# NiteshBharadwaj/pytorch-unsup-pc

Measured on AMD Instinct MI355X. Metric: point-clouds/sec (8000 pts->64^3->128^2 proj) fwd+bwd, higher is better.
Workload: dtype f32

## Files before the change

pytorch-unsup-pc_amd/csrc/dpc_common.h:

```cpp
#pragma once
#include <hip/hip_runtime.h>
#include <stdint.h>

#include "../../include/dpc_render.h"

#define DPC_WAVE 64

template <int RB>
struct TapsT {
  float w[2 * RB + 1];
};

struct TapsDyn {
  float w[DPC_MAX_TAPS];
  int n;
};

template <int RB>
__device__ inline TapsT<RB> resolve_taps(const TapsT<RB>& host, const float* __restrict__ dev, int n, bool flip) {
  if (dev == nullptr || n <= 0) return host;
  TapsT<RB> t;
  const int c = (n - 1) / 2;
#pragma unroll
  for (int i = 0; i < 2 * RB + 1; ++i) {
// ... 94 lines not shown
  for (int i = 0; i < 9; ++i) g.m[i] = 0.f;
  g.dt[0] = g.dt[1] = g.dt[2] = 0.f;
  g.df = 0.f;
}

__device__ inline void project_point_bwd(const Camera& c, const Projected& o, float px, float py, float pz, float dZ,
                                         float dY, float dX, float& dpx, float& dpy, float& dpz, CamGrad& g) {
  const float g2 = c.f * o.inv * dX;
  const float g1 = c.f * o.inv * dY;
  const float persp = -(o.X * dX + o.Y * dY) * o.inv;
  const float g0 = dZ + persp;
  g.df += (o.p2 * dX + o.p1 * dY) * o.inv;
  g.dt[0] += persp;
  g.dt[1] += g1;
  g.dt[2] += g2;
  dpx = fmaf(c.r[0], g0, fmaf(c.r[3], g1, c.r[6] * g2));
  dpy = fmaf(c.r[1], g0, fmaf(c.r[4], g1, c.r[7] * g2));
  dpz = fmaf(c.r[2], g0, fmaf(c.r[5], g1, c.r[8] * g2));
  g.m[0] += px * g0; g.m[1] += px * g1; g.m[2] += px * g2;
  g.m[3] += py * g0; g.m[4] += py * g1; g.m[5] += py * g2;
  g.m[6] += pz * g0; g.m[7] += pz * g1; g.m[8] += pz * g2;
}

__device__ inline void quaternion_grad(const Camera& c, const float* m, float* dq) {
  const float w = c.qw, vx = c.qx, vy = c.qy, vz = c.qz;
  const float tr = m[0] + m[4] + m[8];
  const float cx = m[5] - m[7], cy = m[6] - m[2], cz = m[1] - m[3];
  const float sx = 2.f * m[0] * vx + (m[1] + m[3]) * vy + (m[2] + m[6]) * vz;
  const float sy = (m[3] + m[1]) * vx + 2.f * m[4] * vy + (m[5] + m[7]) * vz;
  const float sz = (m[6] + m[2]) * vx + (m[7] + m[5]) * vy + 2.f * m[8] * vz;
  const float gw = 2.f * (w * tr + vx * cx + vy * cy + vz * cz);
  const float gx = 2.f * (-tr * vx + sx + w * cx);
  const float gy = 2.f * (-tr * vy + sy + w * cy);
  const float gz = 2.f * (-tr * vz + sz + w * cz);
  const float dot = w * gw + vx * gx + vy * gy + vz * gz;
  dq[0] = (gw - w * dot) * c.inv_norm;
  dq[1] = (gx - vx * dot) * c.inv_norm;
  dq[2] = (gy - vy * dot) * c.inv_norm;
  dq[3] = (gz - vz * dot) * c.inv_norm;
}

struct CameraRef {
  float w, x, y, z;
  double cw, cx, cy, cz;
  double tx, ty, tz;
  double f, d;
  bool has_t;
};

__device__ inline CameraRef load_camera_ref(const DpcParams& P, const float* __restrict__ q,
                                            const float* __restrict__ t, const float* __restrict__ f, int b) {
#pragma clang fp contract(off)
  CameraRef c;
  const float q0 = q[4 * b + 0], q1 = q[4 * b + 1], q2 = q[4 * b + 2], q3 = q[4 * b + 3];
  float acc = 0.f;
  acc = acc + q0 * q0;
  acc = acc + q1 * q1;
  acc = acc + q2 * q2;
  acc = acc + q3 * q3;
  const float n = sqrtf(acc);
  c.w = q0 / n; c.x = q1 / n; c.y = q2 / n; c.z = q3 / n;
  c.cw = (double)c.w; c.cx = -(double)c.x; c.cy = -(double)c.y; c.cz = -(double)c.z;
  c.has_t = t != nullptr;
  c.tx = t ? (double)t[3 * b + 0] : 0.0;
  c.ty = t ? (double)t[3 * b + 1] : 0.0;
  c.tz = t ? (double)t[3 * b + 2] : 0.0;
  c.f = f ? (double)f[b] : (double)P.focal_length;
  c.d = (double)P.camera_distance;
  return c;
}

__device__ inline void project_point_ref(const CameraRef& c, float x2, float y2, float z2, double& Z, double& Y,
                                         double& X) {
#pragma clang fp contract(off)
  const float w2 = 0.0f;
  const float w1 = c.w, x1 = c.x, y1 = c.y, z1 = c.z;
  const float aw = ((w1 * w2 - x1 * x2) - y1 * y2) - z1 * z2;
  const float ax = ((w1 * x2 + x1 * w2) + y1 * z2) - z1 * y2;
  const float ay = ((w1 * y2 + y1 * w2) + z1 * x2) - x1 * z2;
  const float az = ((w1 * z2 + z1 * w2) + x1 * y2) - y1 * x2;
  const double dw = (double)aw, dx = (double)ax, dy = (double)ay, dz = (double)az;
  double p0 = ((dw * c.cx + dx * c.cw) + dy * c.cz) - dz * c.cy;
  double p1 = ((dw * c.cy + dy * c.cw) + dz * c.cx) - dx * c.cz;
  double p2 = ((dw * c.cz + dz * c.cw) + dx * c.cy) - dy * c.cx;
  if (c.has_t) {
    p0 = p0 + c.tx; p1 = p1 + c.ty; p2 = p2 + c.tz;
  }
  double zs = p0 + c.d;
  const double xs = (p2 * c.f) / zs;
  const double ys = (p1 * c.f) / zs;
  zs = zs - c.d;
  if (c.has_t) zs = zs - c.tx;
  Z = zs; Y = ys; X = xs;
}

struct __attribute__((aligned(16))) PointRec {
  int code;
  float tz, ty, tx;
};

struct Cell {
  int iz, iy, ix;
  float wz[2], wy[2], wx[2];
  bool valid;
};

__device__ inline float frac_encode(double g, int& cell) {
#pragma clang fp contract(off)
  const double fl = floor(g);
  cell = (int)fl;
  const double r = g - fl;
  return (float)(r < 0.5 ? r : r - 1.0);
}

__device__ inline PointRec make_record(double Z, double Y, double X, int D, int H, int W) {
#pragma clang fp contract(off)
  PointRec rec;
  const bool valid = (Z >= -0.5) && (Z <= 0.5) && (Y >= -0.5) && (Y <= 0.5) && (X >= -0.5) && (X <= 0.5);
  int iz, iy, ix;
  rec.tz = frac_encode((Z + 0.5) * (double)(D - 1), iz);
  rec.ty = frac_encode((Y + 0.5) * (double)(H - 1), iy);
  rec.tx = frac_encode((X + 0.5) * (double)(W - 1), ix);
  rec.code = valid ? ((iz << 20) | (iy << 10) | ix) : -1;
  if (!valid) rec.tz = rec.ty = rec.tx = 0.f;
  return rec;
}

__device__ inline void frac_decode(float t, float (&w)[2]) {
  w[1] = t >= 0.f ? t : 1.0f + t;
  w[0] = t >= 0.f ? 1.0f - t : -t;
}

__device__ inline Cell cell_from_record(const PointRec& rec) {
  Cell c;
  c.valid = rec.code >= 0;
  c.iz = rec.code >> 20;
  c.iy = (rec.code >> 10) & 1023;
  c.ix = rec.code & 1023;
  frac_decode(rec.tz, c.wz);
  frac_decode(rec.ty, c.wy);
  frac_decode(rec.tx, c.wx);
  return c;
}

__device__ inline PointRec load_record(const PointRec* __restrict__ recs, size_t i) {
  const int4 v = *reinterpret_cast<const int4*>(recs + i);
  PointRec r;
  r.code = v.x;
  r.tz = __int_as_float(v.y);
  r.ty = __int_as_float(v.z);
  r.tx = __int_as_float(v.w);
  return r;
}

template <int RB, int L, bool CLAMP1>
__device__ inline void window_load(float (&v)[L + 2 * RB], const float* base, int stride, int start, int len) {
#pragma unroll
  for (int i = 0; i < L + 2 * RB; ++i) {
    const int pos = start + i - RB;
    float x = (pos >= 0 && pos < len) ? base[pos * stride] : 0.f;
    if (CLAMP1) x = fminf(x, 1.0f);
    v[i] = x;
  }
}

template <int RB>
__host__ __device__ constexpr int tap_edge_first(int i) { return i < 2 * RB ? ((i & 1) ? 2 * RB - (i >> 1) : (i >> 1)) : RB; }

template <int RB, int L>
__device__ inline float window_dot(const float (&v)[L + 2 * RB], const TapsT<RB>& taps, int j) {
  float acc = 0.f;
#pragma unroll
  for (int t = 0; t < 2 * RB + 1; ++t) acc = fmaf(taps.w[t], v[j + t], acc);
  return acc;
}

static __global__ __launch_bounds__(256) void k_zero_words(unsigned int* __restrict__ p, size_t n) {
  for (size_t i = (size_t)blockIdx.x * blockDim.x + threadIdx.x; i < n; i += (size_t)gridDim.x * blockDim.x) p[i] = 0u;
}
inline bool zero_words_async(void* p, size_t words, hipStream_t st) {
  if (words == 0) return true;
  const unsigned blocks = (unsigned)((words + 255) / 256 < 2048 ? (words + 255) / 256 : 2048);
  hipLaunchKernelGGL(k_zero_words, dim3(blocks), dim3(256), 0, st, static_cast<unsigned int*>(p), words);
  return hipGetLastError() == hipSuccess;
}

template <int CTRL>
__device__ inline float dpp_move(float v) {
  return __int_as_float(__builtin_amdgcn_update_dpp(0, __float_as_int(v), CTRL, 0xf, 0xf, false));
}

__device__ inline float pooled_mask(const float* __restrict__ masks, int f, int smp, int H, int W, int pix) {
  if (f == 1) return masks[(size_t)smp * H * W + pix];
  const int py = pix / W, px = pix - py * W, Wm = f * W;
  const float* m = masks + ((size_t)smp * H + py) * f * Wm + (size_t)px * f;
  float acc = 0.f;
  for (int i = 0; i < f; ++i)
    for (int j = 0; j < f; ++j) acc += m[(size_t)i * Wm + j];
  return acc / (float)(f * f);
}

__device__ inline float sample_weight2(const float* __restrict__ weights, int smp) {
  if (weights == nullptr) return 1.0f;
  const float w = weights[smp];
  return w * w;
}

__device__ inline float wave_sum(float v) {
  v += dpp_move<0xb1>(v);
  v += dpp_move<0x4e>(v);
  v += dpp_move<0x124>(v);
  v += dpp_move<0x128>(v);
  v += dpp_move<0x142>(v);
  v += dpp_move<0x143>(v);
  return __int_as_float(__builtin_amdgcn_readlane(__float_as_int(v), 63));
}

template <int CTRL, int ROW_MASK>
__device__ inline int dpp_move_int(int v) {
  return __builtin_amdgcn_update_dpp(0, v, CTRL, ROW_MASK, 0xf, false);
}
__device__ inline int wave_inclusive_scan(int v) {
  v += dpp_move_int<0x111, 0xf>(v);
  v += dpp_move_int<0x112, 0xf>(v);
  v += dpp_move_int<0x114, 0xf>(v);
  v += dpp_move_int<0x118, 0xf>(v);
  v += dpp_move_int<0x142, 0xa>(v);
  v += dpp_move_int<0x143, 0xc>(v);
  return v;
}

template <int NV>
__device__ inline void block_sum(float (&vals)[NV], float* red) {
  static_assert(NV <= DPC_WAVE, "one lane per value");
  const int lane = threadIdx.x & (DPC_WAVE - 1), wave = threadIdx.x / DPC_WAVE, nw = (blockDim.x + DPC_WAVE - 1) / DPC_WAVE;
#pragma unroll
  for (int i = 0; i < NV; ++i) vals[i] = wave_sum(vals[i]);
  if (lane == 0) {
#pragma unroll
    for (int i = 0; i < NV; ++i) red[wave * NV + i] = vals[i];
  }
  __syncthreads();
  if (wave == 0) {
    float s = 0.f;
    if (lane < NV)
      for (int k = 0; k < nw; ++k) s += red[k * NV + lane];
#pragma unroll
    for (int i = 0; i < NV; ++i) vals[i] = __shfl(s, i, DPC_WAVE);
  }
}

__host__ __device__ constexpr size_t camgrad_scratch_bytes(int nthr) { return (size_t)13 * (nthr / DPC_WAVE) * sizeof(float); }

__device__ inline double block_sum13_fixed(const float (&vals)[13], float* scratch, int tid, int nthr, int nvals = 13) {
  const int lane = tid & (DPC_WAVE - 1), wave = tid / DPC_WAVE, nw = nthr / DPC_WAVE;
  float ws[13];
#pragma unroll
  for (int i = 0; i < 9; ++i) ws[i] = wave_sum(vals[i]);
  if (nvals > 9) {
#pragma unroll
    for (int i = 9; i < 13; ++i) ws[i] = wave_sum(vals[i]);
  } else {
#pragma unroll
    for (int i = 9; i < 13; ++i) ws[i] = 0.f;
  }
  if (lane == 0) {
#pragma unroll
    for (int i = 0; i < 13; ++i) scratch[wave * 13 + i] = ws[i];
  }
  __syncthreads();
  double tot = 0.0;
  if (tid < 13)
    for (int k = 0; k < nw; ++k) tot += (double)scratch[k * 13 + tid];
  return tot;
}

__device__ inline void quaternion_grad_f64(const float* q_raw, const double* m, double* dq) {
  double w = q_raw[0], vx = q_raw[1], vy = q_raw[2], vz = q_raw[3];
  const double inv_norm = 1.0 / sqrt(w * w + vx * vx + vy * vy + vz * vz);
  w *= inv_norm; vx *= inv_norm; vy *= inv_norm; vz *= inv_norm;
  const double tr = m[0] + m[4] + m[8];
  const double cx = m[5] - m[7], cy = m[6] - m[2], cz = m[1] - m[3];
  const double sx = 2.0 * m[0] * vx + (m[1] + m[3]) * vy + (m[2] + m[6]) * vz;
  const double sy = (m[3] + m[1]) * vx + 2.0 * m[4] * vy + (m[5] + m[7]) * vz;
  const double sz = (m[6] + m[2]) * vx + (m[7] + m[5]) * vy + 2.0 * m[8] * vz;
  const double gw = 2.0 * (w * tr + vx * cx + vy * cy + vz * cz);
  const double gx = 2.0 * (-tr * vx + sx + w * cx);
  const double gy = 2.0 * (-tr * vy + sy + w * cy);
  const double gz = 2.0 * (-tr * vz + sz + w * cz);
  const double dot = w * gw + vx * gx + vy * gy + vz * gz;
  dq[0] = (gw - w * dot) * inv_norm;
  dq[1] = (gx - vx * dot) * inv_norm;
  dq[2] = (gy - vy * dot) * inv_norm;
  dq[3] = (gz - vz * dot) * inv_norm;
}
```

pytorch-unsup-pc_amd/csrc/dpc_kernels.h:

```cpp
#pragma once
#include <math.h>
#include <string.h>

#include <atomic>

#include "dpc_common.h"
#include "dpc_profile.h"

#ifdef DPC_ABLATE
static __device__ int g_dpc_ablate = 0;
#define DPC_ABL(bit) (g_dpc_ablate & (1 << (bit)))
static __device__ unsigned long long* g_dpc_stamps = nullptr;
#define DPC_STAMP(slot)                                                                                    \
  do {                                                                                                     \
    if (g_dpc_stamps != nullptr && threadIdx.x == 0)                                                       \
      g_dpc_stamps[(size_t)blockIdx.x * 16 + (slot)] = __builtin_amdgcn_s_memrealtime(); \
  } while (0)
#define DPC_DEBUG_SETTERS(tag)                                                                                          \
  extern "C" int dpc_debug_set_ablate_##tag(int v) {                                                                    \
    return hipMemcpyToSymbol(HIP_SYMBOL(g_dpc_ablate), &v, sizeof(int)) == hipSuccess ? 0 : -5;                         \
  }                                                                                                                     \
  extern "C" int dpc_debug_set_stamps_##tag(void* p) {                                                                  \
    return hipMemcpyToSymbol(HIP_SYMBOL(g_dpc_stamps), &p, sizeof(void*)) == hipSuccess ? 0 : -5;                       \
  }
#else
#define DPC_ABL(bit) 0
#define DPC_STAMP(slot) do { } while (0)
#define DPC_DEBUG_SETTERS(tag)
#endif

namespace dpck {

constexpr int kSlabThreads = 1024;
constexpr int kColThreads = 256;
constexpr int kNumCUs = 256;
struct SseFormat {
  int frac;
  int cshift;
  int bits;
};
constexpr float kTileSseCap = 4096.0f;
inline int bit_width(unsigned long long v) {
  int n = 0;
  while (v) { ++n; v >>= 1; }
  return n;
}
inline SseFormat sse_format(unsigned long long contributors, double max_share) {
  SseFormat f;
  f.bits = bit_width(contributors);
  f.cshift = 64 - 2 * f.bits;
  const int int_bits = bit_width((unsigned long long)(contributors * max_share) + 1);
  f.frac = f.cshift - int_bits;
  if (f.frac > 30) f.frac = 30;
  if (f.frac < 0) f.frac = 0;
  return f;
}
__device__ inline unsigned long long sse_share(const SseFormat& f, double value, double cap) {
  const bool bad = !(value >= 0.0 && value <= cap);
  return (1ull << f.cshift) | (bad ? (1ull << (f.cshift + f.bits)) : (unsigned long long)(value * (double)(1ull << f.frac) + 0.5));
}
__device__ inline bool sse_complete(const SseFormat& f, unsigned long long before, int contributors) {
  return (int)((before >> f.cshift) & ((1ull << f.bits) - 1ull)) == contributors - 1;
}
__device__ inline double sse_total(const SseFormat& f, unsigned long long word) {
  if ((word >> (f.cshift + f.bits)) != 0ull) return __longlong_as_double(0x7ff8000000000000ll);
  return (double)(word & ((1ull << f.cshift) - 1ull)) * (1.0 / (double)(1ull << f.frac));
}
#ifndef DPC_ZFB_RPL
#define DPC_ZFB_RPL 1
#endif
constexpr int kLocThreads = 256;
constexpr int kL = 16;
constexpr int kLdsLimit = 160 * 1024;
constexpr int kRedTab = 256;
constexpr int kRedMask = 400;
constexpr int kRedFloats = 1024;
constexpr int kLdsBudget = kLdsLimit - 4096;

struct Blk {
  int x, y;
  int nx, ny;
};
__device__ inline Blk block_coords(int clouds, int group = 1) {
  Blk k;
  k.ny = clouds;
  k.nx = (int)gridDim.x / clouds;
  const int L = blockIdx.x;
#ifndef DPC_NO_XCD_MAP
  if (group > 1 && clouds % (8 * group) == 0) {
    const int q = L >> 3, j = q / k.nx;
    k.y = ((L & 7) + 8 * (j / group)) * group + j % group;
    k.x = q % k.nx;
    return k;
  }
  if ((clouds & 7) == 0) {
    const int q = L >> 3;
    k.y = (L & 7) + 8 * (q / k.nx);
    k.x = q % k.nx;
    return k;
  }
#endif
  k.y = L / k.nx;
  k.x = L - k.y * k.nx;
  return k;
}

__host__ __device__ inline int points_per_set(const DpcParams& P) { return P.point_index != nullptr ? P.N_src : P.N; }

__device__ inline int odd_stride(int w) { return w | 1; }

__host__ __device__ inline size_t chunk_bytes(int D) {
  return (size_t)kLocThreads * 2 * sizeof(PointRec) + (((size_t)(D + 2) * 2 + 15) / 16) * 16;
}
__host__ __device__ inline int num_chunks(int N) { return (N + kLocThreads - 1) / kLocThreads; }

struct Cells {
  const uint8_t* base;
  size_t chunk;
  int nblk;
  __device__ const uint8_t* at(int b, int blk) const { return base + ((size_t)b * nblk + blk) * chunk; }
  __device__ const PointRec* recs(int b, int blk) const { return reinterpret_cast<const PointRec*>(at(b, blk)); }
  __device__ const int4* aux(int b, int blk) const {
    return reinterpret_cast<const int4*>(at(b, blk) + (size_t)kLocThreads * sizeof(PointRec));
  }
  __device__ const uint16_t* offs(int b, int blk) const {
    return reinterpret_cast<const uint16_t*>(at(b, blk) + (size_t)kLocThreads * 2 * sizeof(PointRec));
  }
};

constexpr int kTabInts = 2 * DPC_WAVE + 2;

struct RecordRange {
  int beg, cnt;
};

__device__ inline RecordRange load_record_range(const Cells& cells, int b, int bin_lo, int bin_hi) {
  RecordRange r{0, 0};
  const int c = threadIdx.x;
  if (c < DPC_WAVE && c < cells.nblk) {
    const uint16_t* offs = cells.offs(b, c);
    r.beg = offs[bin_lo];
    r.cnt = (int)offs[bin_hi] - r.beg;
  }
  return r;
}

__device__ inline void finish_record_table(const RecordRange& r, int* tab) {
  if (threadIdx.x >= DPC_WAVE) return;
  const int c = threadIdx.x;
  const int incl = wave_inclusive_scan(r.cnt);
  tab[c] = incl - r.cnt;
  tab[DPC_WAVE + 1 + c] = r.beg;
  if (c == DPC_WAVE - 1) tab[DPC_WAVE] = incl;
}

__device__ inline void flat_lookup(const int* tab, int j, int& chunk, int& pos) {
  int lo = 0, hi = DPC_WAVE;
#pragma unroll
  for (int step = 0; step < 6; ++step) {
    const int mid = (lo + hi) >> 1;
    if (tab[mid] <= j) lo = mid; else hi = mid;
  }
  chunk = lo;
  pos = tab[DPC_WAVE + 1 + lo] + (j - tab[lo]);
}

template <class F>
__device__ inline void for_each_record_flat(const Cells& cells, int b, const int* tab, F f, int first = 0) {
  const int total = tab[DPC_WAVE];
  for (int j = first + threadIdx.x; j < total; j += blockDim.x) {
    int c, pos;
    flat_lookup(tab, j, c, pos);
    f(load_record(cells.recs(b, c), pos), cells.aux(b, c) + pos);
  }
}

template <class F>
__device__ inline void for_each_record(const Cells& cells, int b, int bin_lo, int bin_hi, F f) {
  const int lane = threadIdx.x & (DPC_WAVE - 1), wave = threadIdx.x / DPC_WAVE, nw = blockDim.x / DPC_WAVE;
  for (int blk = wave; blk < cells.nblk; blk += nw) {
    const uint16_t* offs = cells.offs(b, blk);
    const int beg = __builtin_amdgcn_readfirstlane((int)offs[bin_lo]);
    const int end = __builtin_amdgcn_readfirstlane((int)offs[bin_hi]);
    const PointRec* recs = cells.recs(b, blk);
    const int4* aux = cells.aux(b, blk);
    for (int j = beg + lane; j < end; j += DPC_WAVE) f(load_record(recs, j), aux + j);
  }
}

template <int RB, bool CLAMP1, class Post>
__device__ inline void wpass_inplace(float* slab, int nz, int H, int W, int WP, const TapsT<RB>& taps, Post post) {
  const int nseg = (W + kL - 1) / kL;
  const int lines = nz * H;
  const int per_round = blockDim.x / nseg;
  for (int l0 = 0; l0 < lines; l0 += per_round) {
    const int li = threadIdx.x % per_round, seg = threadIdx.x / per_round;
    const int line = l0 + li;
    const bool act = seg < nseg && line < lines;
    float v[kL + 2 * RB];
    if (act) window_load<RB, kL, CLAMP1>(v, slab + line * WP, 1, seg * kL, W);
    __syncthreads();
    if (act) {
#pragma unroll
      for (int j = 0; j < kL; ++j) {
        const int x = seg * kL + j;
        if (x < W) slab[line * WP + x] = post(line, x, window_dot<RB, kL>(v, taps, j));
      }
    }
    __syncthreads();
  }
}

template <int RB, class Store>
__device__ inline void hpass(float* slab, int nz, int H, int W, int WP, const TapsT<RB>& taps, Store store) {
  const int nseg = (H + kL - 1) / kL;
  const int lines = nz * W;
  const int per_round = blockDim.x / nseg;
  for (int l0 = 0; l0 < lines; l0 += per_round) {
    const int li = threadIdx.x % per_round, seg = threadIdx.x / per_round;
    const int line = l0 + li;
    const bool act = seg < nseg && line < lines;
    const int z = line / W, x = line - z * W;
    float v[kL + 2 * RB];
    if (act) window_load<RB, kL, false>(v, slab + z * H * WP + x, WP, seg * kL, H);
    __syncthreads();
    if (act) {
#pragma unroll
      for (int j = 0; j < kL; ++j) {
        const int y = seg * kL + j;
        if (y < H) store(z, y, x, window_dot<RB, kL>(v, taps, j));
      }
    }
    __syncthreads();
  }
}

typedef float f32x2 __attribute__((ext_vector_type(2)));
typedef float f32x4 __attribute__((ext_vector_type(4)));

__device__ inline void store_through(float* p, float v) { __hip_atomic_store(p, v, __ATOMIC_RELAXED, __HIP_MEMORY_SCOPE_AGENT); }
__device__ inline void store_through(f32x2* p, f32x2 v) {
  __hip_atomic_store(reinterpret_cast<unsigned long long*>(p), __builtin_bit_cast(unsigned long long, v), __ATOMIC_RELAXED,
                     __HIP_MEMORY_SCOPE_AGENT);
}
constexpr int kAuxThrough = 16;

#ifndef DPC_BWD_NARROW_PAD
#define DPC_BWD_NARROW_PAD 1
#endif
constexpr bool kBwdNarrowPad = DPC_BWD_NARROW_PAD != 0;
#ifndef DPC_BWD_ZS64
#define DPC_BWD_ZS64 8
#endif
constexpr int kBwdZs64 = DPC_BWD_ZS64;

template <int GS, int RB, int NT_, int LW_, int LH_, int PADO = -1>
struct SlabGeo {
  static constexpr int PAD = PADO >= 0 ? PADO : (RB <= 4 ? 4 : ((RB + 3) / 4) * 4);
  static constexpr bool NARROW = PAD < RB;
  static constexpr int LEAD = NARROW ? ((RB + 1 - PAD + 3) / 4) * 4 : 0;
  static constexpr int WP = GS + PAD;
  static constexpr int WPA = GS + PAD + 2;
  static constexpr int PLANE = GS * WP;
  static constexpr int LW = LW_, NSEGW = GS / LW, LWIN = LW + 2 * PAD;
  static constexpr int LH = LH_, NSEGH = GS / LH, XP = GS / 2, HWIN = LH + 2 * RB;
  static constexpr int NT = NT_;
  __host__ __device__ static constexpr size_t slab_floats(int planes) { return (size_t)planes * PLANE + PAD + 2 * LEAD; }
  __device__ static int at(int z, int y, int x) { return LEAD + (z * GS + y) * WP + PAD + x; }
  __device__ static int row_start(int row) { return LEAD + row * WP; }
};
template <int GS, int ZS, int RB>
using FwdGeo = SlabGeo<GS, RB, ZS * GS * GS / 16, 16, 8>;
constexpr int bwd_threads(int gs, int npl) {
  const int items = npl * gs * (gs / 32);
  return items >= 1024 ? 1024 : (items <= 256 ? 256 : ((items + 63) / 64) * 64);
}
template <int GS, int RB, int NPL>
using BwdGeo = SlabGeo<GS, RB, bwd_threads(GS, NPL), 32, (GS == 128 ? 8 : 16), (GS == 64 && RB > 4 && NPL == kBwdZs64 + 1 && kBwdNarrowPad ? 4 : -1)>;

constexpr float kFixScale = 17592186044416.0f;
constexpr float kFixInv = 1.0f / 17592186044416.0f;
constexpr unsigned long long kFixOne = 1ull << 44;
static_assert((unsigned long long)DPC_MAX_POINTS <= ~0ull / kFixOne, "DPC_MAX_POINTS unit weights must fit the 64-bit accumulator");

__device__ inline unsigned long long to_fixed(float w) {
  const float scaled = w * 4096.0f;
  const unsigned int hi = (unsigned int)scaled;
  const float rem = scaled - (float)hi;
  const unsigned int lo = (unsigned int)(rem * 4294967296.0f);
  return ((unsigned long long)hi << 32) | lo;
}
__device__ inline float from_fixed(unsigned long long a) {
  unsigned int hi = (unsigned int)(a >> 32), lo = (unsigned int)a;
  asm("" : "+v"(hi), "+v"(lo));
  return fmaf((float)hi, 0x1p-12f, (float)lo * kFixInv);
}

template <class Geo, int GS, int NPL>
__host__ __device__ constexpr int wpass_items_per_thread() {
  return (NPL * GS * Geo::NSEGW + Geo::NT - 1) / Geo::NT;
}

template <class Geo, int GS, int NPL>
__device__ inline void wpass_mask_prefetch(const uint32_t* __restrict__ mask32, int planes_present,
                                           uint32_t (&bits)[wpass_items_per_thread<Geo, GS, NPL>()]) {
  constexpr int ROWS = NPL * GS, ITEMS = ROWS * Geo::NSEGW, IPT = wpass_items_per_thread<Geo, GS, NPL>();
#pragma unroll
  for (int it = 0; it < IPT; ++it) {
    const int item = threadIdx.x + it * Geo::NT;
    bits[it] = 0u;
    if (item < ITEMS) {
      const int row = item % ROWS, seg = item / ROWS;
      if (row / GS < planes_present) bits[it] = mask32[(size_t)row * Geo::NSEGW + seg];
    }
  }
}

template <class Geo, int GS, int RB, int NPL, bool CLAMP1, int MASK>
__device__ inline void wpass_fast(float* slab, const TapsT<RB>& taps, const uint32_t* mask32, int planes_present) {
  constexpr int ROWS = NPL * GS, ITEMS = ROWS * Geo::NSEGW, IPT = (ITEMS + Geo::NT - 1) / Geo::NT;
  float v[IPT][Geo::LWIN];
#pragma unroll
  for (int it = 0; it < IPT; ++it) {
    const int item = threadIdx.x + it * Geo::NT;
    if (item < ITEMS) {
      const int row = item % ROWS, seg = item / ROWS;
// ... 455 lines not shown
```

pytorch-unsup-pc_amd/csrc/dpc_slab_bwd.hip:

```cpp
#include "dpc_kernels.h"

DPC_DEBUG_SETTERS(bwd)

namespace dpck {
namespace {

template <int GS, int ZS, int RB>
__global__ __launch_bounds__(kSlabThreads) void k_gather_hw(DpcParams P, Cells cells, const float* __restrict__ pc,
                                                            const float* __restrict__ q, const float* __restrict__ t,
                                                            const float* __restrict__ f, TapsT<RB> taps_arg, int zs_rt,
                                                            const float* __restrict__ dT,
                                                            const uint64_t* __restrict__ mask,
                                                            const float* __restrict__ ds_part, int n_ds_part,
                                                            float* __restrict__ dpc, float* __restrict__ dsmall,
                                                            double* __restrict__ cg_part,
                                                            unsigned int* __restrict__ cg_count, LossArgs la,
                                                            unsigned long long* __restrict__ dpc_fixed) {
  extern __shared__ __attribute__((aligned(16))) float slab[];
  const TapsT<RB> taps_adj = resolve_taps<RB>(taps_arg, P.dev_taps_xy, P.taps_xy, true);
  const int D = P.D, H = P.H, W = P.W, HW = H * W;
  const int Zs = GS ? ZS : zs_rt;
  constexpr bool kRolls = GS > 0 && ZS == 1 && RB > 0;
  const int roll = kRolls ? zs_rt : 1;
  const int reps = P.point_replicas > 1 ? P.point_replicas : 1;
  const bool shared_points = reps > 1 || P.point_index != nullptr;
  const bool wo = winners_only(la) && shared_points;
  const bool single_writer = wo && reps == la.K && P.point_index == nullptr;
  const Blk bk = block_coords(wo ? P.B / la.K : P.B, la.winner != nullptr ? la.K : 1);
  const int b = wo ? bk.y * la.K + la.winner[bk.y] : bk.y, z0 = bk.x * Zs * roll;
  const int Nset = points_per_set(P);
  if (cloud_loses(la, b)) {
    if (shared_points) {
      if (bk.x == 0 && threadIdx.x == 0) dsmall[(size_t)DPC_COL_DS * P.B + b] = 0.f;
      return;
    }
    float* dz = dpc + (size_t)b * Nset * 3;
    auto zero3 = [&](const PointRec&, const int4* aux) {
      const int i = aux->w;
      dz[3 * i + 0] = 0.f; dz[3 * i + 1] = 0.f; dz[3 * i + 2] = 0.f;
    };
    for_each_record(cells, b, z0, min(z0 + Zs * roll, D), zero3);
    if (bk.x == 0) {
      for_each_record(cells, b, D, D + 1, zero3);
      if (threadIdx.x == 0) dsmall[(size_t)DPC_COL_DS * P.B + b] = 0.f;
    }
    return;
  }
  const bool down = kRolls && (bk.x & 1);
  const int zfirst = down ? min(z0 + roll, D) - 1 : z0;
  const int nzp = min(Zs + 1, D - zfirst);
  const int tid = threadIdx.x, nthr = blockDim.x;
  const CameraRaw cam_raw = load_camera_raw(P, q, t, f, b);
  const float upstream = (la.scale_in_gather && la.dloss != nullptr) ? *la.dloss : 1.0f;
  const int wpp = (HW + 63) / 64;
  const float* src = dT + ((size_t)b * D + zfirst) * HW;
  const uint64_t* mrow = mask + ((size_t)b * D + zfirst) * wpp;
  float* red;

  if constexpr (GS > 0) {
    constexpr int NPL = ZS + 1;
    using Geo = BwdGeo<GS, RB, NPL>;
    red = slab + ((Geo::slab_floats(NPL) + 3) / 4) * 4;
    RecordRange rr{0, 0};
    if (cells.nblk <= DPC_WAVE) rr = load_record_range(cells, b, zfirst, min(zfirst + Zs, D));
    const uint32_t* mask32 = reinterpret_cast<const uint32_t*>(mrow);
    DPC_STAMP(8);
    for (int i = tid; i < (NPL * GS + 1) * (Geo::PAD / 4); i += Geo::NT) {
      const int p4 = i % (Geo::PAD / 4), row = i / (Geo::PAD / 4);
      *reinterpret_cast<f32x4*>(slab + Geo::row_start(row) + 4 * p4) = f32x4{0.f, 0.f, 0.f, 0.f};
    }
    if constexpr (Geo::NARROW)
      if (tid < 2 * Geo::LEAD) slab[tid < Geo::LEAD ? tid : Geo::row_start(NPL * GS) + Geo::PAD + tid - Geo::LEAD] = 0.f;
    if constexpr (RB == 0) {
      for (int i = tid; i < NPL * GS * (GS / 4); i += Geo::NT) {
        const int x4 = i % (GS / 4), zy = i / (GS / 4);
        f32x4 val = f32x4{0.f, 0.f, 0.f, 0.f};
        if (zy < nzp * GS) val = *reinterpret_cast<const f32x4*>(src + (size_t)zy * GS + 4 * x4);
        *reinterpret_cast<f32x4*>(slab + Geo::row_start(zy) + Geo::PAD + 4 * x4) = val;
      }
      if (cells.nblk <= DPC_WAVE) finish_record_table(rr, reinterpret_cast<int*>(red + kRedTab));
      __syncthreads();
      const float w2 = taps_adj.w[0] * taps_adj.w[0];
      for (int i = tid; i < NPL * GS * GS; i += Geo::NT) {
        const int x = i % GS, zy = i / GS;
        const bool pass = zy < nzp * GS && ((mask32[i >> 5] >> (i & 31)) & 1u);
        float* cell = slab + Geo::row_start(zy) + Geo::PAD + x;
        *cell = pass ? w2 * *cell : 0.f;
      }
      __syncthreads();
    } else {
      constexpr int MW = NPL * GS * (GS / 32), MPT = (MW + Geo::NT - 1) / Geo::NT;
      uint32_t mreg[MPT];
#pragma unroll
      for (int it = 0; it < MPT; ++it) {
        const int w = tid + it * Geo::NT;
        mreg[it] = (w < MW && w / (GS * (GS / 32)) < nzp) ? mask32[w] : 0u;
      }
      hpass_global<Geo, GS, RB, NPL>(src, nzp, taps_adj, [&](int z, int y, int x, f32x2 val) {
        *reinterpret_cast<f32x2*>(slab + Geo::at(z, y, x)) = val;
      });
      uint32_t* mlds = reinterpret_cast<uint32_t*>(red + kRedMask);
#pragma unroll
      for (int it = 0; it < MPT; ++it) {
        const int w = tid + it * Geo::NT;
        if (w < MW) mlds[w] = mreg[it];
      }
      if (cells.nblk <= DPC_WAVE) finish_record_table(rr, reinterpret_cast<int*>(red + kRedTab));
      __syncthreads();
      DPC_STAMP(9);
      DPC_STAMP(10);
    }
  } else {
    const int WP = odd_stride(W);
    red = slab + (size_t)(Zs + 1) * H * WP;
    for (int i = tid; i < nzp * HW; i += nthr) {
      const int x = i % W, zy = i / W;
      slab[zy * WP + x] = src[i];
    }
    __syncthreads();
    if (RB == 0) {
      const float w2 = taps_adj.w[0] * taps_adj.w[0];
      for (int i = tid; i < nzp * HW; i += nthr) {
        const int z = i / HW, r = i - z * HW;
        const int x = r % W, y = r / W;
        const bool pass = (mrow[(size_t)z * wpp + (r >> 6)] >> (r & 63)) & 1ull;
        slab[(z * H + y) * WP + x] = pass ? w2 * slab[(z * H + y) * WP + x] : 0.f;
      }
      __syncthreads();
    } else {
      hpass<RB>(slab, nzp, H, W, WP, taps_adj, [&](int z, int y, int x, float val) { slab[(z * H + y) * WP + x] = val; });
      wpass_inplace<RB, false>(slab, nzp, H, W, WP, taps_adj, [&](int line, int x, float val) {
        const int z = line / H, y = line - z * H;
        const int bit = y * W + x;
        return ((mrow[(size_t)z * wpp + (bit >> 6)] >> (bit & 63)) & 1ull) ? val : 0.f;
      });
    }
  }

  if (DPC_ABL(12)) return;
  const Camera cam = make_camera(P, cam_raw);
  CamGrad g;
  camgrad_zero(g);
  float* dcloud = dpc + (size_t)(b / reps) * Nset * 3;
  auto corner = [&](int zz, int yy, int xx) -> float {
    if constexpr (GS > 0) return slab[BwdGeo<GS, RB, ZS + 1>::at(zz, yy, xx)];
    else return slab[(zz * H + yy) * odd_stride(W) + xx];
  };
  auto reaches_over = [](int pos) constexpr {
    constexpr int P4 = BwdGeo<(GS > 0 ? GS : 64), RB, ZS + 1>::PAD;
    return pos < RB - P4 || pos >= RB + P4 + 1;
  };
  auto masked_taps = [&](const Cell& c, float (&wm)[2][2 * RB + 1]) {
    constexpr int P4 = BwdGeo<(GS > 0 ? GS : 64), RB, ZS + 1>::PAD;
#pragma unroll
    for (int pos = 0; pos < 2 * RB + 2; ++pos) {
      if (!reaches_over(pos)) continue;
      const bool inside = pos < RB - P4 ? c.ix >= RB - pos : c.ix <= GS - 1 + RB - pos;
      if (pos <= 2 * RB) wm[0][pos] = inside ? taps_adj.w[pos] : 0.f;
      if (pos >= 1) wm[1][pos - 1] = inside ? taps_adj.w[pos - 1] : 0.f;
    }
  };
  auto corner_row = [&](const Cell& c, int k, int j, float& o0, float& o1, const float (&wm)[2][2 * RB + 1]) {
    if constexpr (GS > 0 && RB > 0) {
      using Geo = BwdGeo<GS, RB, ZS + 1>;
      const uint32_t* mlds = reinterpret_cast<const uint32_t*>(red + kRedMask);
      o0 = o1 = 0.f;
      if ((c.iz + k < D) && (c.iy + j < GS)) {
        const int plane = kRolls ? ((c.iz - zfirst + k) & 1) : (c.iz - z0 + k);
        const int row = plane * GS + c.iy + j;
        const float* rp = slab + Geo::row_start(row) + Geo::PAD + c.ix - RB;
        float v[2 * RB + 2];
#pragma unroll
        for (int i = 0; i < 2 * RB + 2; ++i) v[i] = rp[i];
        float o[2];
#pragma unroll
        for (int e = 0; e < 2; ++e) {
          float acc = 0.f;
#pragma unroll
          for (int i = 0; i < 2 * RB + 1; ++i) {
            const int tp = tap_edge_first<RB>(i);
            if (Geo::NARROW && reaches_over(e + tp)) acc = fmaf(wm[e][tp], v[e + tp], acc);
            else acc = fmaf(taps_adj.w[tp], v[e + tp], acc);
          }
          const int x = c.ix + e;
          const bool pass = x < GS && ((mlds[row * (GS / 32) + (x >> 5)] >> (x & 31)) & 1u);
          o[e] = pass ? acc : 0.f;
        }
        o0 = o[0]; o1 = o[1];
      }
    }
  };
  auto finish_point = [&](const int4 pt, float dgz, float dgy, float dgx) {
    const int i = pt.w;
    dgz *= upstream; dgy *= upstream; dgx *= upstream;
    const float px = __int_as_float(pt.x), py = __int_as_float(pt.y), pz = __int_as_float(pt.z);
    const Projected o = project_point(cam, px, py, pz);
    float dpx, dpy, dpz;
    project_point_bwd(cam, o, px, py, pz, dgz * (float)(D - 1), dgy * (float)(H - 1), dgx * (float)(W - 1), dpx, dpy, dpz, g);
    if (shared_points && !single_writer) {
      if (grad_fits_fixed(dpx, dpy, dpz)) {
        unsigned long long* acc = dpc_fixed + ((size_t)(b / reps) * Nset + i) * 3;
        atomicAdd(acc + 0, grad_to_fixed(dpx)); atomicAdd(acc + 1, grad_to_fixed(dpy)); atomicAdd(acc + 2, grad_to_fixed(dpz));
      } else {
        atomicOr(reinterpret_cast<unsigned int*>(dpc_fixed + (size_t)(P.B / reps) * Nset * 3) + b / reps, 1u);
      }
    } else {
      dcloud[3 * i + 0] = dpx; dcloud[3 * i + 1] = dpy; dcloud[3 * i + 2] = dpz;
    }
  };
  auto gather = [&](const PointRec& rec, const int4* aux) {
    const int4 pt = *aux;
    const Cell c = cell_from_record(rec);
    float cv[2][2][2];
    if constexpr (GS > 0 && RB > 0) {
      float wm[2][2 * RB + 1];
      if constexpr (BwdGeo<GS, RB, ZS + 1>::NARROW) masked_taps(c, wm);
#pragma unroll
      for (int k = 0; k < 2; ++k)
#pragma unroll
        for (int j = 0; j < 2; ++j) corner_row(c, k, j, cv[k][j][0], cv[k][j][1], wm);
    } else {
#pragma unroll
      for (int k = 0; k < 2; ++k)
#pragma unroll
        for (int j = 0; j < 2; ++j)
#pragma unroll
          for (int e = 0; e < 2; ++e) {
            const bool ok = (c.iz + k < D) && (c.iy + j < H) && (c.ix + e < W);
            cv[k][j][e] = ok ? corner(c.iz - z0 + k, c.iy + j, c.ix + e) : 0.f;
          }
    }
    float dgz = 0.f, dgy = 0.f, dgx = 0.f;
#pragma unroll
    for (int a = 0; a < 2; ++a)
#pragma unroll
      for (int e = 0; e < 2; ++e) {
        dgz += (cv[1][a][e] - cv[0][a][e]) * c.wy[a] * c.wx[e];
        dgy += (cv[a][1][e] - cv[a][0][e]) * c.wz[a] * c.wx[e];
        dgx += (cv[a][e][1] - cv[a][e][0]) * c.wz[a] * c.wy[e];
      }
    finish_point(pt, dgz, dgy, dgx);
  };
  if (!DPC_ABL(10)) {
    if (GS > 0 && cells.nblk <= DPC_WAVE) for_each_record_flat(cells, b, reinterpret_cast<const int*>(red + kRedTab), gather);
    else for_each_record(cells, b, zfirst, min(zfirst + Zs, D), gather);
  }
  if constexpr (kRolls) {
    using Geo = BwdGeo<GS, RB, 2>;
    constexpr int MW1 = GS * (GS / 32), MPT1 = (MW1 + Geo::NT - 1) / Geo::NT;
    const uint32_t* mask32 = reinterpret_cast<const uint32_t*>(mrow);
    uint32_t* mlds = reinterpret_cast<uint32_t*>(red + kRedMask);
    int* tab = reinterpret_cast<int*>(red + kRedTab);
    const bool flat = cells.nblk <= DPC_WAVE;
    for (int l = 1; l < roll && (down ? zfirst - l >= z0 : z0 + l < D); ++l) {
      __syncthreads();
      const int zl = down ? zfirst - l : z0 + l;
      const int znew = down ? zl : zl + 1;
      const int buf = (znew - zfirst) & 1;
      const bool present = znew < D;
      RecordRange rr{0, 0};
      if (flat) rr = load_record_range(cells, b, zl, zl + 1);
      const ptrdiff_t rel = (ptrdiff_t)znew - zfirst;
      uint32_t mreg[MPT1];
#pragma unroll
      for (int it = 0; it < MPT1; ++it) {
        const int w = tid + it * Geo::NT;
        mreg[it] = (w < MW1 && present) ? mask32[rel * MW1 + w] : 0u;
      }
      hpass_global<Geo, GS, RB, 1>(src + rel * HW, present ? 1 : 0, taps_adj, [&](int, int y, int x, f32x2 val) {
        *reinterpret_cast<f32x2*>(slab + Geo::at(buf, y, x)) = val;
      });
#pragma unroll
      for (int it = 0; it < MPT1; ++it) {
        const int w = tid + it * Geo::NT;
        if (w < MW1) mlds[buf * MW1 + w] = mreg[it];
      }
      if (flat) finish_record_table(rr, tab);
      __syncthreads();
      if (flat) for_each_record_flat(cells, b, tab, gather);
      else for_each_record(cells, b, zl, zl + 1, gather);
    }
  }
  DPC_STAMP(11);
  if (bk.x == 0 && !shared_points)
    for_each_record(cells, b, D, D + 1, [&](const PointRec&, const int4* aux) {
      const int i = aux->w;
      dcloud[3 * i + 0] = 0.f; dcloud[3 * i + 1] = 0.f; dcloud[3 * i + 2] = 0.f;
    });

  float vals[13];
#pragma unroll
  for (int i = 0; i < 9; ++i) vals[i] = g.m[i];
  vals[9] = g.dt[0]; vals[10] = g.dt[1]; vals[11] = g.dt[2]; vals[12] = g.df;
  if (DPC_ABL(13)) { if (vals[0] == 123.f) dsmall[0] = vals[1]; return; }
  const double tot = block_sum13_fixed(vals, red, tid, nthr, (t != nullptr || f != nullptr) ? 13 : 9);
  DPC_STAMP(12);
  if (tid == 0 && bk.x == 0) {
    float ds = 0.f;
    for (int i = 0; i < n_ds_part; ++i) ds += ds_part[(size_t)b * n_ds_part + i];
    dsmall[(size_t)DPC_COL_DS * P.B + b] = ds * upstream;
  }
  camgrad_publish(tot, tid, cam_raw, P.B, b, bk.x, bk.nx, cg_part, cg_count, dsmall, t != nullptr, f != nullptr);
  DPC_STAMP(13);
}

__global__ __launch_bounds__(256) void k_fixed_to_dpc(const unsigned long long* __restrict__ acc, float* __restrict__ dpc, size_t n,
                                                       size_t per_set) {
  const unsigned int* poison = reinterpret_cast<const unsigned int*>(acc + n);
  for (size_t i = (size_t)blockIdx.x * blockDim.x + threadIdx.x; i < n; i += (size_t)gridDim.x * blockDim.x)
    dpc[i] = poison[i / per_set] != 0u ? __int_as_float(0x7fc00000) : dpc[i] + (float)((double)(long long)acc[i] * kGradFixInv);
}

bool fixed_point_gradients(const DpcParams* p, const LossArgs& la) {
  const bool shared = p->point_replicas > 1 || p->point_index != nullptr;
  const int reps = p->point_replicas > 1 ? p->point_replicas : 1;
  const bool single_writer = winners_only(la) && shared && reps == la.K && p->point_index == nullptr;
  return shared && !single_writer;
}

template <int GS, int ZS, int RB>
int launch_gather_fast(const DpcParams* p, Cells cells, const float* pc, const float* q, const float* t, const float* f,
                       const float* kxy, const TapPlan& pxy, const float* dT, const uint64_t* mask,
                       const float* ds_part, int ntile, float* dpc, float* dsmall, double* cg_part, unsigned int* cg_count,
                       const LossArgs& la, hipStream_t st, unsigned long long* dpc_fixed) {
  using Geo = BwdGeo<GS, RB, ZS + 1>;
  constexpr size_t lds = (((Geo::slab_floats(ZS + 1) + 3) / 4) * 4 + kRedMask + (ZS + 1) * GS * (GS / 32)) * sizeof(float);
  static_assert(lds <= kLdsLimit, "backward slab does not fit LDS");
  static_assert(kRedTab >= 13 * (Geo::NT / DPC_WAVE) && kRedMask >= kRedTab + kTabInts, "scratch tail layout");
  auto kern = k_gather_hw<GS, ZS, RB>;
  static LdsLimit limit;
  int rc = set_lds(kern, lds, limit);
  if (rc != DPC_OK) return rc;
  const bool wo = winners_only(la) && (p->point_replicas > 1 || p->point_index != nullptr);
  const int clouds = wo ? p->B / la.K : p->B;
  int roll = 1;
  if (ZS == 1 && RB > 0)
    for (int c = 2; c <= 16; c *= 2)
      if (p->D % c == 0 && (size_t)(p->D / c) * clouds >= (size_t)kNumCUs) roll = c;
  const int nslab = (p->D + ZS - 1) / ZS;
  DPC_LAUNCH("k_gather_hw", dpc_kid("k_gather_hw", GS, ZS, RB), kern, dim3(((nslab + roll - 1) / roll) * clouds), dim3(Geo::NT), lds, st, *p, cells, pc, q, t, f,
             make_taps<RB>(kxy, pxy, true), ZS == 1 ? roll : ZS, dT, mask, ds_part, ntile, dpc, dsmall, cg_part, cg_count, la, dpc_fixed);
  return launch_ok();
}

template <int RB>
int launch_gather_rb(const DpcParams* p, Cells cells, const float* pc, const float* q, const float* t, const float* f,
                  const float* kxy, const TapPlan& pxy, const float* dT, const uint64_t* mask, const float* ds_part,
                  int ntile, float* dpc, float* dsmall, double* cg_part, unsigned int* cg_count, const LossArgs& la,
                  hipStream_t st, unsigned long long* dpc_fixed) {
  if (p->H == p->W) {
    const bool wo64 = winners_only(la) && (p->point_replicas > 1 || p->point_index != nullptr);
    const bool thick = (size_t)(wo64 ? p->B / la.K : p->B) * ((p->D + kBwdZs64 - 1) / kBwdZs64) >= (size_t)kNumCUs;
    if constexpr (RB <= 4) {
      if (p->H == 32) return launch_gather_fast<32, 4, RB>(p, cells, pc, q, t, f, kxy, pxy, dT, mask, ds_part, ntile, dpc, dsmall, cg_part, cg_count, la, st, dpc_fixed);
      if (p->H == 128) return launch_gather_fast<128, 1, RB>(p, cells, pc, q, t, f, kxy, pxy, dT, mask, ds_part, ntile, dpc, dsmall, cg_part, cg_count, la, st, dpc_fixed);
      if (p->H == 64 && thick) return launch_gather_fast<64, kBwdZs64, RB>(p, cells, pc, q, t, f, kxy, pxy, dT, mask, ds_part, ntile, dpc, dsmall, cg_part, cg_count, la, st, dpc_fixed);
      if (p->H == 64) return launch_gather_fast<64, kBwdZs64Thin, RB>(p, cells, pc, q, t, f, kxy, pxy, dT, mask, ds_part, ntile, dpc, dsmall, cg_part, cg_count, la, st, dpc_fixed);
    } else if constexpr (RB <= 10) {
      if constexpr (kBwdNarrowPad)
        if (p->H == 64 && thick) return launch_gather_fast<64, kBwdZs64, RB>(p, cells, pc, q, t, f, kxy, pxy, dT, mask, ds_part, ntile, dpc, dsmall, cg_part, cg_count, la, st, dpc_fixed);
      if (p->H == 64) return launch_gather_fast<64, kBwdZs64Wide, RB>(p, cells, pc, q, t, f, kxy, pxy, dT, mask, ds_part, ntile, dpc, dsmall, cg_part, cg_count, la, st, dpc_fixed);
      if (p->H == 128) return launch_gather_fast<128, 1, RB>(p, cells, pc, q, t, f, kxy, pxy, dT, mask, ds_part, ntile, dpc, dsmall, cg_part, cg_count, la, st, dpc_fixed);
      if (p->H == 32) return launch_gather_fast<32, 4, RB>(p, cells, pc, q, t, f, kxy, pxy, dT, mask, ds_part, ntile, dpc, dsmall, cg_part, cg_count, la, st, dpc_fixed);
    }
  }
  const int fit = planes_fit(p);
  if (fit < 2) return DPC_ERR_LDS;
  const int Zs = std::min(fit - 1, std::max(1, (p->D + 7) / 8));
  const size_t lds = ((size_t)(Zs + 1) * p->H * (p->W | 1) + kRedFloats) * sizeof(float);
  auto kern = k_gather_hw<0, 0, RB>;
  static LdsLimit limit;
  int rc = set_lds(kern, lds, limit);
  if (rc != DPC_OK) return rc;
  const bool wo = winners_only(la) && (p->point_replicas > 1 || p->point_index != nullptr);
  DPC_LAUNCH("k_gather_hw", dpc_kid("k_gather_hw", 0, 0, RB), kern, dim3(((p->D + Zs - 1) / Zs) * (wo ? p->B / la.K : p->B)), dim3(slab_threads(p)), lds, st, *p, cells, pc, q, t, f,
             make_taps<RB>(kxy, pxy, true), Zs, dT, mask, ds_part, ntile, dpc, dsmall, cg_part, cg_count, la, dpc_fixed);
  return launch_ok();
}

}

int launch_gather(int bucket, const DpcParams* p, Cells cells, const float* pc, const float* q, const float* t, const float* f,
                  const float* kxy, const TapPlan& pxy, const float* dT, const uint64_t* mask, const float* ds_part, int ntile,
                  float* dpc, float* dsmall, double* cg_part, unsigned int* cg_count, const LossArgs& la, hipStream_t st,
                  unsigned long long* dpc_fixed) {
  const bool fixed = fixed_point_gradients(p, la) && p->N > 0;
  const int reps = p->point_replicas > 1 ? p->point_replicas : 1;
  const size_t nfix = (size_t)(p->B / reps) * points_per_set(*p) * 3;
  if (fixed) {
    if (dpc_fixed == nullptr) return DPC_ERR_NULL;
    if (!zero_words_async(dpc_fixed, 2 * nfix + (size_t)(p->B / reps), st)) return DPC_ERR_LAUNCH;
  }
  int rc = DPC_OK;
#define DPC_GATHER(RB) rc = launch_gather_rb<RB>(p, cells, pc, q, t, f, kxy, pxy, dT, mask, ds_part, ntile, dpc, dsmall, cg_part, cg_count, la, st, dpc_fixed)
  DPC_FOR_BUCKET(bucket, DPC_GATHER)
#undef DPC_GATHER
  if (rc != DPC_OK || !fixed) return rc;
// ... 6 lines not shown
```

Measured before the change: 608,900.

## Add lean GS=64 gather path with precomputed flat lookups and fused corner rows

For the 64-grid backward gather with small blur radius, the first two record offsets per thread are precomputed right after the record table is built, using a two-level coarse/fine search instead of a binary search. Records are then addressed by byte offset. A specialized corner_rows routine loads each slab row window once and reads the 64-bit mask word directly from LDS. The upstream scale is skipped when it equals 1, and gradient stores use byte-offset addressing. This cuts index arithmetic and LDS lookups per point, at the cost of more code and extra register pressure from the template specialization.

```diff
diff --git a/pytorch-unsup-pc_amd/csrc/dpc_common.h b/pytorch-unsup-pc_amd/csrc/dpc_common.h
--- a/pytorch-unsup-pc_amd/csrc/dpc_common.h
+++ b/pytorch-unsup-pc_amd/csrc/dpc_common.h
@@ -270,6 +270,9 @@
   r.tx = __int_as_float(v.w);
   return r;
 }
+__device__ inline PointRec load_record_at(const uint8_t* __restrict__ base, uint32_t byte_off) {
+  return load_record(reinterpret_cast<const PointRec*>(base + byte_off), 0);
+}
 
 template <int RB, int L, bool CLAMP1>
 __device__ inline void window_load(float (&v)[L + 2 * RB], const float* base, int stride, int start, int len) {
diff --git a/pytorch-unsup-pc_amd/csrc/dpc_kernels.h b/pytorch-unsup-pc_amd/csrc/dpc_kernels.h
--- a/pytorch-unsup-pc_amd/csrc/dpc_kernels.h
+++ b/pytorch-unsup-pc_amd/csrc/dpc_kernels.h
@@ -172,6 +172,55 @@
     int c, pos;
     flat_lookup(tab, j, c, pos);
     f(load_record(cells.recs(b, c), pos), cells.aux(b, c) + pos);
+  }
+}
+
+struct FlatPair {
+  uint32_t off[2];
+};
+template <int NT>
+__device__ inline FlatPair flat_lookup_pair(const int* tab, uint32_t chunk_bytes32) {
+  FlatPair p{{0u, 0u}};
+  const int total = tab[DPC_WAVE];
+  const int j0 = threadIdx.x;
+  if (j0 >= total) return p;
+  int coarse[7];
+#pragma unroll
+  for (int m = 0; m < 7; ++m) coarse[m] = tab[8 * (m + 1)];
+  auto find = [&](int j) -> uint32_t {
+    int c0 = 0;
+#pragma unroll
+    for (int m = 0; m < 7; ++m) c0 += coarse[m] <= j ? 8 : 0;
+    const int4 lo = *reinterpret_cast<const int4*>(tab + c0), hi = *reinterpret_cast<const int4*>(tab + c0 + 4);
+    const int fine[7] = {lo.y, lo.z, lo.w, hi.x, hi.y, hi.z, hi.w};
+    int c = c0;
+#pragma unroll
+    for (int m = 0; m < 7; ++m) c += fine[m] <= j ? 1 : 0;
+    const int pos = tab[DPC_WAVE + 1 + c] + (j - tab[c]);
+    return (uint32_t)c * chunk_bytes32 + (uint32_t)pos * (uint32_t)sizeof(PointRec);
+  };
+  p.off[0] = find(j0);
+  if (j0 + NT < total) p.off[1] = find(j0 + NT);
+  return p;
+}
+
+template <int NT, class F>
+__device__ inline void for_each_record_flat(const Cells& cells, int b, const int* tab, const FlatPair& pre, F f) {
+  const int total = tab[DPC_WAVE];
+  const uint8_t* base = cells.at(b, 0);
+  const uint8_t* aux_base = base + (size_t)kLocThreads * sizeof(PointRec);
+  const uint32_t chunk_bytes32 = (uint32_t)cells.chunk;
+  int round = 0;
+  for (int j = threadIdx.x; j < total; j += NT, ++round) {
+    uint32_t off;
+    if (round < 2) {
+      off = round == 0 ? pre.off[0] : pre.off[1];
+    } else {
+      int c, pos;
+      flat_lookup(tab, j, c, pos);
+      off = (uint32_t)c * chunk_bytes32 + (uint32_t)pos * (uint32_t)sizeof(PointRec);
+    }
+    f(load_record_at(base, off), reinterpret_cast<const int4*>(aux_base + off));
   }
 }
 
diff --git a/pytorch-unsup-pc_amd/csrc/dpc_slab_bwd.hip b/pytorch-unsup-pc_amd/csrc/dpc_slab_bwd.hip
--- a/pytorch-unsup-pc_amd/csrc/dpc_slab_bwd.hip
+++ b/pytorch-unsup-pc_amd/csrc/dpc_slab_bwd.hip
@@ -1,4 +1,5 @@
 #include "dpc_kernels.h"
+#include <type_traits>
 
 DPC_DEBUG_SETTERS(bwd)
 
@@ -22,6 +23,7 @@
   const int Zs = GS ? ZS : zs_rt;
   constexpr bool kRolls = GS > 0 && ZS == 1 && RB > 0;
   const int roll = kRolls ? zs_rt : 1;
+  constexpr bool kLean = GS == 64 && RB > 0 && RB <= 4;
   const int reps = P.point_replicas > 1 ? P.point_replicas : 1;
   const bool shared_points = reps > 1 || P.point_index != nullptr;
   const bool wo = winners_only(la) && shared_points;
@@ -56,6 +58,7 @@
   const float* src = dT + ((size_t)b * D + zfirst) * HW;
   const uint64_t* mrow = mask + ((size_t)b * D + zfirst) * wpp;
   float* red;
+  [[maybe_unused]] FlatPair pre{{0u, 0u}};
 
   if constexpr (GS > 0) {
     constexpr int NPL = ZS + 1;
@@ -107,6 +110,8 @@
       }
       if (cells.nblk <= DPC_WAVE) finish_record_table(rr, reinterpret_cast<int*>(red + kRedTab));
       __syncthreads();
+      if constexpr (kLean)
+        if (cells.nblk <= DPC_WAVE) pre = flat_lookup_pair<Geo::NT>(reinterpret_cast<const int*>(red + kRedTab), (uint32_t)cells.chunk);
       DPC_STAMP(9);
       DPC_STAMP(10);
     }
@@ -190,9 +195,51 @@
       }
     }
   };
+  auto corner_rows = [&](const Cell& c, float (&cv)[2][2][2], const float (&wm)[2][2 * RB + 1]) {
+    if constexpr (kLean) {
+      using Geo = BwdGeo<GS, RB, ZS + 1>;
+      const int plane = c.iz - z0;
+      const int row00 = plane * GS + c.iy;
+      const int win = Geo::row_start(row00) + Geo::PAD + c.ix - RB;
+      const bool next_row = c.iy + 1 < GS;
+      const int dj = next_row ? 1 : 0;
+      constexpr int dk = GS;
+      const uint32_t* mlds = reinterpret_cast<const uint32_t*>(red + kRedMask);
+      const int mw = row00 * (GS / 32);
+#pragma unroll
+      for (int k = 0; k < 2; ++k)
+#pragma unroll
+        for (int j = 0; j < 2; ++j) {
+          const int drow = k * dk + j * dj;
+          int wi = win + drow * Geo::WP, mi = mw + drow * (GS / 32);
+          asm volatile("" : "+v"(wi), "+v"(mi));
+          const float* rp = slab + wi;
+          float v[2 * RB + 2];
+#pragma unroll
+          for (int i = 0; i < 2 * RB + 2; ++i) v[i] = rp[i];
+          const uint64_t word = *reinterpret_cast<const uint64_t*>(mlds + mi);
+          uint32_t bits = (uint32_t)(word >> c.ix);
+          if (j == 1) bits = next_row ? bits : 0u;
+          const bool pass[2] = {(bits & 1u) != 0u, (bits & 2u) != 0u};
+#pragma unroll
+          for (int e = 0; e < 2; ++e) {
+            float acc = 0.f;
+#pragma unroll
+            for (int i = 0; i < 2 * RB + 1; ++i) {
+              const int tp = tap_edge_first<RB>(i);
+              if (Geo::NARROW && reaches_over(e + tp)) acc = fmaf(wm[e][tp], v[e + tp], acc);
+              else acc = fmaf(taps_adj.w[tp], v[e + tp], acc);
+            }
+            cv[k][j][e] = pass[e] ? acc : 0.f;
+          }
+          if (k + j < 2) __builtin_amdgcn_sched_barrier(0);
+        }
+    }
+  };
+  const bool scaled = !kLean || upstream != 1.0f;
   auto finish_point = [&](const int4 pt, float dgz, float dgy, float dgx) {
     const int i = pt.w;
-    dgz *= upstream; dgy *= upstream; dgx *= upstream;
+    if (scaled) { dgz *= upstream; dgy *= upstream; dgx *= upstream; }
     const float px = __int_as_float(pt.x), py = __int_as_float(pt.y), pz = __int_as_float(pt.z);
     const Projected o = project_point(cam, px, py, pz);
     float dpx, dpy, dpz;
@@ -205,20 +252,29 @@
         atomicOr(reinterpret_cast<unsigned int*>(dpc_fixed + (size_t)(P.B / reps) * Nset * 3) + b / reps, 1u);
       }
     } else {
-      dcloud[3 * i + 0] = dpx; dcloud[3 * i + 1] = dpy; dcloud[3 * i + 2] = dpz;
-    }
-  };
-  auto gather = [&](const PointRec& rec, const int4* aux) {
+      if constexpr (kLean) {
+        float* dp = reinterpret_cast<float*>(reinterpret_cast<uint8_t*>(dcloud) + (uint32_t)i * 12u);
+        dp[0] = dpx; dp[1] = dpy; dp[2] = dpz;
+      } else {
+        dcloud[3 * i + 0] = dpx; dcloud[3 * i + 1] = dpy; dcloud[3 * i + 2] = dpz;
+      }
+    }
+  };
+  auto gather_rows = [&](auto lean_rows, const PointRec& rec, const int4* aux) {
     const int4 pt = *aux;
     const Cell c = cell_from_record(rec);
     float cv[2][2][2];
     if constexpr (GS > 0 && RB > 0) {
       float wm[2][2 * RB + 1];
       if constexpr (BwdGeo<GS, RB, ZS + 1>::NARROW) masked_taps(c, wm);
-#pragma unroll
-      for (int k = 0; k < 2; ++k)
-#pragma unroll
-        for (int j = 0; j < 2; ++j) corner_row(c, k, j, cv[k][j][0], cv[k][j][1], wm);
+      if constexpr (decltype(lean_rows)::value) {
+        corner_rows(c, cv, wm);
+      } else {
+#pragma unroll
+        for (int k = 0; k < 2; ++k)
+#pragma unroll
+          for (int j = 0; j < 2; ++j) corner_row(c, k, j, cv[k][j][0], cv[k][j][1], wm);
+      }
     } else {
 #pragma unroll
       for (int k = 0; k < 2; ++k)
@@ -241,8 +297,13 @@
       }
     finish_point(pt, dgz, dgy, dgx);
   };
+  auto gather = [&](const PointRec& rec, const int4* aux) { gather_rows(std::false_type{}, rec, aux); };
+  [[maybe_unused]] auto gather_lean = [&](const PointRec& rec, const int4* aux) { gather_rows(std::bool_constant<kLean>{}, rec, aux); };
   if (!DPC_ABL(10)) {
-    if (GS > 0 && cells.nblk <= DPC_WAVE) for_each_record_flat(cells, b, reinterpret_cast<const int*>(red + kRedTab), gather);
+    if constexpr (kLean) {
+      if (cells.nblk <= DPC_WAVE) for_each_record_flat<BwdGeo<GS, RB, ZS + 1>::NT>(cells, b, reinterpret_cast<const int*>(red + kRedTab), pre, gather_lean);
+      else for_each_record(cells, b, zfirst, min(zfirst + Zs, D), gather);
+    } else if (GS > 0 && cells.nblk <= DPC_WAVE) for_each_record_flat(cells, b, reinterpret_cast<const int*>(red + kRedTab), gather);
     else for_each_record(cells, b, zfirst, min(zfirst + Zs, D), gather);
   }
   if constexpr (kRolls) {
```

After: 613,300, median of 3. About the same (+0.7%).
